# APRIL-ZJU/Gaussian-LIC

Measured on AMD Instinct MI355X. Metric: rendered views/sec (fwd+bwd) at 1080p, 2M Gaussians, higher is better.
Workload: dtype f32; 1 GPU; BASELINE config 3: 2000000 Gaussians (random scene, seed 0), 1920x1080, SH degree 3, render fwd + 0.8*L1+0.2*(1-fused-SSIM) + bwd + sparse Adam per view (fused entry points: activations and loss inside the kernels); learning rates x0.01 (stationary synthetic scene); map rows kept in Morton order by the library (bit-identical results; `insertion_order` beside it with --extras); mode=train, parallelism=single, math=strict, map_order=morton, binning=atomic (auto)

## Files before the change

### gaussian-lic_amd/_lib.py

```python
import ctypes
import os

import torch

_HERE = os.path.dirname(os.path.abspath(__file__))
LIB_PATH = os.environ.get("GSLIC_HIP_LIB") or os.path.join(_HERE, "libgslic_hip.so")

ALLOC_FN = ctypes.CFUNCTYPE(ctypes.c_void_p, ctypes.c_void_p, ctypes.c_size_t)


class RasterParams(ctypes.Structure):
    _fields_ = [("P", ctypes.c_int32), ("D", ctypes.c_int32), ("M", ctypes.c_int32), ("width", ctypes.c_int32),
                ("height", ctypes.c_int32), ("tan_fovx", ctypes.c_float), ("tan_fovy", ctypes.c_float),
                ("limx_neg", ctypes.c_float), ("limx_pos", ctypes.c_float), ("limy_neg", ctypes.c_float),
                ("limy_pos", ctypes.c_float), ("scale_modifier", ctypes.c_float), ("prefiltered", ctypes.c_int32),
                ("debug", ctypes.c_int32), ("no_color", ctypes.c_int32), ("raw_params", ctypes.c_int32), ("tie_rank", ctypes.c_void_p)]


class AdamGroup(ctypes.Structure):
    _fields_ = [("param", ctypes.c_void_p), ("grad", ctypes.c_void_p), ("exp_avg", ctypes.c_void_p),
                ("exp_avg_sq", ctypes.c_void_p), ("lr", ctypes.c_float), ("M", ctypes.c_uint32)]


class RowArray(ctypes.Structure):
    _fields_ = [("src", ctypes.c_void_p), ("dst", ctypes.c_void_p), ("row_dwords", ctypes.c_uint32)]


class AdamFused(ctypes.Structure):
    _fields_ = [("param", ctypes.c_void_p * 6), ("exp_avg", ctypes.c_void_p * 6), ("exp_avg_sq", ctypes.c_void_p * 6),
                ("lr", ctypes.c_float * 6), ("b1", ctypes.c_float), ("b2", ctypes.c_float), ("eps", ctypes.c_float), ("visible_out", ctypes.c_void_p)]


class GradStats(ctypes.Structure):
    _fields_ = [("grad_sum", ctypes.c_void_p), ("n_seen", ctypes.c_void_p), ("max_radius", ctypes.c_void_p)]


class ExposureAdam(ctypes.Structure):
    _fields_ = [("param", ctypes.c_void_p), ("m", ctypes.c_void_p), ("v", ctypes.c_void_p), ("step_count", ctypes.c_void_p), ("view", ctypes.c_void_p),
                ("lr", ctypes.c_float), ("beta1", ctypes.c_float), ("beta2", ctypes.c_float), ("eps", ctypes.c_float), ("skip", ctypes.c_void_p)]


EXPORTS = [
    "gslic_rasterize_forward", "gslic_rasterize_backward", "gslic_rasterize_backward_adam", "gslic_rasterize_backward_camera", "gslic_adam_update", "gslic_adam_update_groups",
    "gslic_fusedssim_forward", "gslic_fusedssim_backward", "gslic_knn_mean_dist2", "gslic_abi_version",
    "gslic_last_error", "gslic_geom_bytes", "gslic_img_bytes", "gslic_binning_bytes", "gslic_sample_bytes",
    "gslic_profile_enable", "gslic_profile_reset", "gslic_profile_collect", "gslic_profile_num_kernels",
    "gslic_profile_kernel_name", "gslic_profile_get", "gslic_debug_export", "gslic_extend_select", "gslic_extend_emit", "gslic_loss_partials_count", "gslic_l1_ssim_loss_forward", "gslic_l1_ssim_loss_forward_backward",
    "gslic_l1_ssim_loss_backward", "gslic_set_math_mode", "gslic_set_binning_mode", "gslic_rasterize_forward_capacity", "gslic_rasterize_backward_rgb",
    "gslic_rasterize_backward_rgb_rows", "gslic_sh_grad_from_rgb", "gslic_sh_grad_from_rgb_adam", "gslic_rasterize_backward_rgb_payload",
    "gslic_sh_grad_from_rgb_adam_all", "gslic_get_binning_path", "gslic_scratch_round_up",
    "gslic_rasterize_forward_depth", "gslic_rasterize_backward_depth",
    "gslic_rasterize_forward_depth_capacity", "gslic_rasterize_backward_depth_adam", "gslic_depth_l1_loss_partials_count",
    "gslic_depth_l1_loss_forward_backward", "gslic_img_bytes_depth", "gslic_binning_bytes_depth", "gslic_sample_bytes_depth",
    "gslic_rasterize_backward_depth_camera", "gslic_prune_select", "gslic_gather_rows", "gslic_contribution_accumulate",
    "gslic_contribution_accumulate_error", "gslic_contribution_accumulate_free_space", "gslic_densify_select", "gslic_densify_emit",
    "gslic_l1_ssim_loss_weighted_partials_count", "gslic_l1_ssim_loss_weighted_forward_backward",
    "gslic_morton_order", "gslic_permute_rows", "gslic_permute_rows_staging_bytes",
    "gslic_rasterize_backward_adam_stats", "gslic_rasterize_backward_depth_adam_stats", "gslic_gradient_stats_accumulate",
    "gslic_lidar_zbuffer_add", "gslic_lidar_zbuffer_resolve", "gslic_lidar_zbuffer_resolve_weighted",
    "gslic_depth_loss_weighted_partials_count", "gslic_depth_loss_weighted_forward_backward",
    "gslic_geometry_images",
    "gslic_exposure_partials_count", "gslic_exposure_apply", "gslic_exposure_backward",
    "gslic_keyframe_decode", "gslic_keyframe_encode",
]

_lib = None


class GslicError(RuntimeError):
    pass


def lib():
    global _lib
    if _lib is not None:
        return _lib
    if not os.path.exists(LIB_PATH):
        raise GslicError(f"{LIB_PATH} is missing: run `python gaussian-lic_amd/build.py` (hipcc, gfx950). "
                         "There is no CPU fallback.")
    L = ctypes.CDLL(LIB_PATH, mode=ctypes.RTLD_GLOBAL)
    vp, i32, f32, u32 = ctypes.c_void_p, ctypes.c_int32, ctypes.c_float, ctypes.c_uint32
    L.gslic_last_error.restype = ctypes.c_char_p
    L.gslic_profile_kernel_name.restype = ctypes.c_char_p
    L.gslic_profile_kernel_name.argtypes = [i32]
    L.gslic_profile_get.argtypes = [i32, ctypes.POINTER(ctypes.c_double), ctypes.POINTER(ctypes.c_int64)]
    for n in ("gslic_geom_bytes", "gslic_img_bytes", "gslic_binning_bytes", "gslic_sample_bytes", "gslic_img_bytes_depth", "gslic_binning_bytes_depth",
              "gslic_sample_bytes_depth"):
        getattr(L, n).restype = ctypes.c_size_t
    L.gslic_geom_bytes.argtypes = [i32]
    L.gslic_img_bytes.argtypes = [i32, i32]
    L.gslic_binning_bytes.argtypes = [i32, i32]
    L.gslic_sample_bytes.argtypes = [i32]
    L.gslic_img_bytes_depth.argtypes = [i32, i32]
    L.gslic_binning_bytes_depth.argtypes = [i32]
    L.gslic_sample_bytes_depth.argtypes = [i32]
    L.gslic_depth_l1_loss_partials_count.restype = ctypes.c_int64
    L.gslic_depth_l1_loss_partials_count.argtypes = [i32, i32]
    L.gslic_depth_l1_loss_forward_backward.argtypes = [i32, i32, f32, vp, vp, vp, vp, vp, vp]
    L.gslic_depth_loss_weighted_partials_count.restype = ctypes.c_int64
    L.gslic_depth_loss_weighted_partials_count.argtypes = [i32, i32]
    L.gslic_depth_loss_weighted_forward_backward.argtypes = [i32, i32, f32, f32] + [vp] * 6 + [vp]
    L.gslic_exposure_partials_count.restype = ctypes.c_int64
    L.gslic_exposure_partials_count.argtypes = [i32, i32]
    L.gslic_exposure_apply.argtypes = [i32, i32, vp, vp, vp, vp]
    L.gslic_exposure_backward.argtypes = [i32, i32] + [vp] * 6 + [ctypes.POINTER(ExposureAdam), vp]
    L.gslic_keyframe_decode.argtypes = [i32, i32, i32, vp, vp, vp, i32, vp, vp, vp]
    L.gslic_keyframe_encode.argtypes = [i32, i32, vp, vp, vp, vp, i32, i32, vp]
    prm, counts, adam = ctypes.POINTER(RasterParams), [ctypes.POINTER(i32), ctypes.POINTER(i32)], ctypes.POINTER(AdamFused)
    inputs = [vp] * 12
    fwd_head = [prm] + [ALLOC_FN, vp] * 4 + inputs
    cap_head = [prm] + [vp, ctypes.c_size_t] * 4 + inputs
    bwd_head = [prm, i32, i32] + inputs + [vp] * 4
    ten, six, five = [vp] * 10 + [f32], [vp] * 6 + [f32], [vp] * 5 + [f32]
    L.gslic_rasterize_forward.argtypes = fwd_head + [vp] * 3 + counts + [vp]
    L.gslic_rasterize_forward_depth.argtypes = fwd_head + [vp] * 4 + counts + [vp]
    L.gslic_rasterize_forward_capacity.argtypes = cap_head + [vp] * 3 + counts + [vp, vp]
    L.gslic_rasterize_forward_depth_capacity.argtypes = cap_head + [vp] * 4 + counts + [vp, vp]
    L.gslic_rasterize_backward.argtypes = bwd_head + [vp] + ten + [vp]
    L.gslic_rasterize_backward_depth.argtypes = bwd_head + [vp, vp] + ten + [vp]
    L.gslic_rasterize_backward_adam.argtypes = bwd_head + [vp] + six + [adam, vp]
    L.gslic_rasterize_backward_depth_adam.argtypes = bwd_head + [vp, vp] + six + [adam, vp]
    gstats = ctypes.POINTER(GradStats)
    L.gslic_rasterize_backward_adam_stats.argtypes = bwd_head + [vp] + six + [adam, gstats, vp]
    L.gslic_rasterize_backward_depth_adam_stats.argtypes = bwd_head + [vp, vp] + six + [adam, gstats, vp]
    L.gslic_gradient_stats_accumulate.argtypes = [i32, vp, vp, gstats, i32, i32, vp]
    L.gslic_rasterize_backward_camera.argtypes = bwd_head + [vp] + ten + [vp] * 3 + [vp]
    L.gslic_rasterize_backward_depth_camera.argtypes = bwd_head + [vp, vp] + ten + [vp] * 3 + [vp]
    L.gslic_rasterize_backward_rgb.argtypes = bwd_head + [vp] + five + [vp]
    L.gslic_rasterize_backward_rgb_rows.argtypes = bwd_head + [vp] + five + [i32, i32, i32, vp]
    L.gslic_rasterize_backward_rgb_payload.argtypes = bwd_head + [vp] + five + [vp, vp, vp]
    L.gslic_sh_grad_from_rgb_adam_all.argtypes = [i32, i32, i32, i32, vp, vp, vp, i32, vp, ctypes.c_int64, vp, ctypes.POINTER(AdamFused), vp, vp, vp, vp,
                                                  ctypes.c_int64, vp]
    L.gslic_sh_grad_from_rgb.argtypes = [i32, i32, i32, i32, vp, vp, vp, i32, vp, vp, ctypes.c_int64, vp]
    L.gslic_sh_grad_from_rgb_adam.argtypes = [i32, i32, i32, i32, vp, vp, vp, i32, vp, ctypes.POINTER(AdamFused), vp, vp, ctypes.c_int64, vp]
    L.gslic_adam_update.argtypes = [vp, vp, vp, vp, vp, f32, f32, f32, f32, u32, u32, vp]
    L.gslic_adam_update_groups.argtypes = [ctypes.POINTER(AdamGroup), i32, vp, f32, f32, f32, u32, vp]
    L.gslic_fusedssim_forward.argtypes = [i32, i32, i32, i32, f32, f32] + [vp] * 6 + [vp]
    L.gslic_fusedssim_backward.argtypes = [i32, i32, i32, i32, f32, f32] + [vp] * 7 + [vp]
    L.gslic_knn_mean_dist2.argtypes = [i32, vp, vp, ALLOC_FN, vp, vp]
    L.gslic_extend_select.argtypes = [i32, vp, vp, vp, vp, f32, f32, f32, f32, i32, i32, vp, ALLOC_FN, vp,
                                      ctypes.POINTER(vp), ctypes.POINTER(vp), ctypes.POINTER(i32), vp]
    L.gslic_extend_emit.argtypes = [i32, vp, vp, vp, vp, vp, f32, f32, i32, vp, vp, vp, vp, vp, vp, vp]
    L.gslic_prune_select.argtypes = [i32, vp, vp, vp, vp, vp, f32, f32, i32, vp, vp, vp, i32, ALLOC_FN, vp, vp, vp,
                                     ctypes.POINTER(i32), ctypes.POINTER(i32), vp]
    L.gslic_gather_rows.argtypes = [ctypes.POINTER(RowArray), i32, vp, i32, vp]
    L.gslic_lidar_zbuffer_add.argtypes = [i32, vp, vp, vp, f32, f32, f32, f32, i32, i32, vp, i32, i32, vp]
    L.gslic_lidar_zbuffer_resolve.argtypes = [i32, i32, vp, i32, f32, f32, vp, vp, vp, vp, vp]
    L.gslic_lidar_zbuffer_resolve_weighted.argtypes = [i32, i32, vp, i32, f32, f32, f32, f32, f32, vp, vp, vp, vp, vp, vp, vp]
    L.gslic_morton_order.argtypes = [i32, vp, vp, ALLOC_FN, vp, vp, vp, vp]
    L.gslic_permute_rows.argtypes = [ctypes.POINTER(RowArray), i32, vp, i32, vp, ctypes.c_size_t, vp]
    L.gslic_permute_rows_staging_bytes.restype = ctypes.c_size_t
    L.gslic_permute_rows_staging_bytes.argtypes = [ctypes.POINTER(RowArray), i32, i32]
    L.gslic_contribution_accumulate.argtypes = [prm, i32, i32, vp, vp, vp, f32, vp, vp, vp, vp]
    L.gslic_contribution_accumulate_error.argtypes = [prm, i32, i32, vp, vp, vp, f32, vp, vp, vp, vp, vp, vp]
    L.gslic_contribution_accumulate_free_space.argtypes = [prm, i32, i32, vp, vp, vp, f32, vp, vp, vp, vp, vp, vp, vp]
    L.gslic_geometry_images.argtypes = [prm, i32, i32, vp, vp, vp, f32] + [vp] * 7 + [vp]
    L.gslic_densify_select.argtypes = [i32, vp, vp, vp, vp, vp, vp, vp, vp, f32, ALLOC_FN, vp, vp, ctypes.POINTER(i32), ctypes.POINTER(i32), vp]
    six_ptrs = ctypes.POINTER(vp)
    L.gslic_densify_emit.argtypes = [i32, i32, vp, i32, six_ptrs, six_ptrs, six_ptrs, vp, f32, u32, vp]
    L.gslic_debug_export.argtypes = [ctypes.POINTER(RasterParams), i32, i32] + [vp] * 4 + [vp] * 10 + [vp]
    L.gslic_loss_partials_count.restype = ctypes.c_int64
    L.gslic_loss_partials_count.argtypes = [i32, i32, i32, i32]
    L.gslic_l1_ssim_loss_forward.argtypes = [i32, i32, i32, i32, f32, f32] + [vp] * 7 + [vp]
    L.gslic_l1_ssim_loss_backward.argtypes = [i32, i32, i32, i32, f32] + [vp] * 6 + [vp]
    L.gslic_l1_ssim_loss_forward_backward.argtypes = [i32, i32, i32, i32, f32, f32, f32] + [vp] * 8 + [vp]
    L.gslic_l1_ssim_loss_weighted_partials_count.restype = ctypes.c_int64
    L.gslic_l1_ssim_loss_weighted_partials_count.argtypes = [i32, i32, i32]
    L.gslic_l1_ssim_loss_weighted_forward_backward.argtypes = [i32, i32, i32, f32, f32, f32] + [vp] * 9 + [vp]
    L.gslic_set_math_mode.argtypes = [i32]
    L.gslic_set_binning_mode.argtypes = [i32]
    L.gslic_get_binning_path.argtypes = [ctypes.POINTER(u32), ctypes.POINTER(u32)]
    L.gslic_scratch_round_up.restype = ctypes.c_size_t
    L.gslic_scratch_round_up.argtypes = [ctypes.c_size_t]
    if L.gslic_abi_version() != 8:
        raise GslicError("libgslic_hip.so ABI version mismatch")
    _lib = L
    return L


def set_math_mode(strict):
    return bool(lib().gslic_set_math_mode(int(bool(strict))))


def set_binning_mode(mode):
    names = ("auto", "radix", "atomic")
    return names[lib().gslic_set_binning_mode(names.index(mode))]


def binning_path():
    a, n = ctypes.c_uint32(0), ctypes.c_uint32(0)
    path = lib().gslic_get_binning_path(ctypes.byref(a), ctypes.byref(n))
    return ("none", "radix", "atomic")[path], a.value, n.value


def check(rc):
    if rc != 0:
        raise GslicError(f"libgslic_hip error {rc}: {lib().gslic_last_error().decode()}")


def ptr(t):
    if t is None or t.numel() == 0:
        return None
    return ctypes.c_void_p(t.data_ptr())


def current_stream_ptr():
    return ctypes.c_void_p(torch.cuda.current_stream().cuda_stream)


class _AllocBox:
    __slots__ = ("device", "tensor", "__weakref__")

    def __init__(self, device):
# ... 57 lines not shown
```

### gaussian-lic_amd/csrc/api.hip

```cpp
#include "gslic_common.h"
#include "kernels.h"
#include <atomic>
#include <chrono>
#include <cmath>
#include <mutex>

#include <stdarg.h>
#include <stdio.h>
#include <stdlib.h>
#include <string.h>
#include <vector>

namespace gslic {

static thread_local char g_err[512] = "";
int set_error(int code, const char* fmt, ...)
{
    va_list ap;
    va_start(ap, fmt);
    vsnprintf(g_err, sizeof(g_err), fmt, ap);
    va_end(ap);
    return code;
}

// ... 506 lines not shown
        if (use_bin) {
            TileBinArgs tb;
            tb.T = T; tb.n_cap = R; tb.n_dev = R_dev; tb.tile = ka.tile_keys; tb.gid = ka.gauss; tb.depth = ka.depth; tb.tie_rank = prm->tie_rank;
            tb.ranges = img.ranges; tb.binned = bin.binned(); tb.dead = bin.dead; tb.status = geom.flags;
            tb.bucket_offsets = no_color ? nullptr : img.bucket_offsets; tb.max_contrib = img.max_contrib;
            ts.long_tiles = reinterpret_cast<uint32_t*>(bin.sort_scratch);
            GS_TRY(launch_tile_bin(tb, s));
            DEBUG_SYNC(prm, s);
            ts.binned = bin.binned(); ts.depth = nullptr; ts.gauss_in = nullptr; ts.slot_in = nullptr;
            ts.key_a = bin.tile_keys[0]; ts.key_b = bin.tile_keys[1]; ts.idx_a = bin.gauss[pp]; ts.idx_b = bin.slots[pp];
        } else {
            SortBuffers sb;
            for (int i = 0; i < 2; i++) { sb.keys[i] = bin.tile_keys[i]; sb.v0[i] = bin.slots[i]; sb.v1[i] = bin.gauss[i]; sb.v2[i] = bin.lsort[i]; }
            sb.v0_identity = true;
            GS_TRY(radix_sort_u32(sb, bin.plan, bin.sort_scratch, (onesweep_mask() & 2) != 0, K_SORT_HIST, K_SORT_SCATTER, s, R_dev, geom.flags + GS_FLAG_FAULT));
            DEBUG_SYNC(prm, s);
            GS_TRY(launch_finalize_ranges(R, R_dev, bin.tile_keys[pp], img.ranges, bin.dead, s));
            DEBUG_SYNC(prm, s);
            ts.binned = nullptr; ts.depth = bin.lsort[pp]; ts.gauss_in = bin.gauss[pp]; ts.slot_in = bin.slots[pp];
            ts.key_a = bin.lsort[pp ^ 1]; ts.key_b = bin.tile_keys[pp ^ 1]; ts.idx_a = bin.lsort[2]; ts.idx_b = bin.lsort[3];
        }
        GS_TRY(launch_tile_depth_sort(ts, s));
        DEBUG_SYNC(prm, s);
    }

    SampleState smp;
    memset(&smp, 0, sizeof(smp));
    uint32_t B = 0;
    if (!no_color) {
        if (!use_bin) GS_TRY(launch_bucket_scan(T, img.ranges, img.bucket_offsets, img.max_contrib, s));
        if (cap) {
            B = capacity_for(cap->sample_bytes, [&](uint32_t b) { size_t n; SampleState::carve(nullptr, (size_t)b, &n, depth); return n; });
        } else {
            uint32_t bin_sample[2] = {0, 0};
            GS_TRY(fetch_counts(img.bucket_offsets + (T - 1), nullptr, hostbuf, s, geom.flags + GS_FLAG_FAULT,
                                use_bin ? geom.flags + GS_FLAG_BIN_ATOMICS : nullptr, bin_sample));
            if (hostbuf[1] & 2u) return set_error(GSLIC_ERR_HIP, "a sort look-back / chained-scan wait timed out (device preempted?): the forward was abandoned");
            B = hostbuf[0];
            binning_feedback(prm->tie_rank != nullptr, use_bin, bin_sample[0], bin_sample[1]);
        }
        size_t smp_bytes;
        SampleState::carve(nullptr, (size_t)B, &smp_bytes, depth);
        char* smp_base = cap ? cap->sample : c.sample_alloc(c.sample_ctx, smp_bytes);
        if (!smp_base) return set_error(GSLIC_ERR_ALLOC, "sample allocator returned NULL for %zu bytes", smp_bytes);
        smp = SampleState::carve(align256(smp_base), (size_t)B, nullptr, depth);
    }

    RenderFwdArgs ra;
    ra.W = prm->width; ra.H = prm->height; ra.gx = gx; ra.gy = gy; ra.no_color = prm->no_color;
    ra.ranges = img.ranges; ra.point_list = bin.point_list(); ra.rec = geom.rec; ra.bucket_offsets = img.bucket_offsets;
    ra.bucket_to_tile = smp.bucket_to_tile; ra.ckpt = smp.ckpt; ra.hit = smp.hit; ra.pix_final = img.pix_final; ra.max_contrib = img.max_contrib;
    ra.out_color = c.out_color; ra.out_final_T = c.out_final_T; ra.capB = B; ra.status = geom.flags; ra.tail4_from = T;
    ra.out_depth = depth ? c.out_depth : nullptr; ra.ckpt_depth = smp.ckpt_depth; ra.pix_depth = img.pix_depth;
    GS_TRY(launch_render_fwd(ra, s));
    note_depth(geom.flags, depth);
    DEBUG_SYNC(prm, s);
    if (cap) {
        hipLaunchKernelGGL(forward_status_kernel, dim3(1), dim3(1), 0, s, (const uint32_t*)(geom.point_offsets + (P - 1)),
                           no_color ? (const uint32_t*)nullptr : (const uint32_t*)(img.bucket_offsets + (T - 1)), geom.flags, geom.flags + GS_FLAG_FAULT,
                           cap->status_out);
        GS_HIP(hipGetLastError());
    }

    *c.num_rendered = (int32_t)R;
    *c.num_buckets = (int32_t)B;
    return GSLIC_OK;
}

extern "C" {
int gslic_set_binning_mode(int32_t mode)
{
    if (mode < 0 || mode > 2) return g_binning_mode.load(std::memory_order_relaxed);
    const int old = g_binning_mode.exchange(mode, std::memory_order_relaxed);
    g_binning_epoch.fetch_add(1u, std::memory_order_release);
    return old;
}
int gslic_get_binning_path(uint32_t* sampled_atomics, uint32_t* sampled_instances)
{
    if (sampled_atomics) *sampled_atomics = t_last_sample[0];
    if (sampled_instances) *sampled_instances = t_last_sample[1];
    return t_last_path;
}
size_t gslic_scratch_round_up(size_t n)
{
    if (n <= (size_t(1) << 20)) return n;
    size_t g = size_t(32) << 20;
    if (n > (size_t(64) << 20)) {
        size_t p = 1;
        while ((p << 1) <= n && (p << 1) != 0) p <<= 1;
        const size_t half = p >> 1, cap = size_t(256) << 20;
        g = half > cap ? cap : (half > g ? half : g);
    }
    return (n + g - 1) / g * g;
}
#define GS_FORWARD_SHARED(c)                                                                                                               \
    c.prm = prm; c.means3D = means3D; c.dc = dc; c.shs = shs; c.colors_precomp = colors_precomp; c.opacities = opacities; c.scales = scales;       \
    c.rotations = rotations; c.cov3D_precomp = cov3D_precomp; c.viewmatrix = viewmatrix; c.projmatrix = projmatrix; c.cam_pos = cam_pos;           \
    c.out_color = out_color; c.out_final_T = out_final_T; c.radii = radii; c.stream = stream
#define GS_FORWARD_ALLOCATORS(c)                                                                                                           \
    c.geom_alloc = geom_alloc; c.geom_ctx = geom_ctx; c.binning_alloc = binning_alloc; c.binning_ctx = binning_ctx; c.img_alloc = img_alloc;       \
    c.img_ctx = img_ctx; c.sample_alloc = sample_alloc; c.sample_ctx = sample_ctx; c.num_rendered = num_rendered; c.num_buckets = num_buckets
#define GS_FORWARD_CAPACITY(c, cap)                                                                                                        \
    const ForwardCapacity cap{geom_buffer, binning_buffer, img_buffer, sample_buffer, geom_bytes, binning_bytes, img_bytes, sample_bytes, status}; \
    c.cap = &cap; c.num_rendered = capacity_R; c.num_buckets = capacity_B

int gslic_rasterize_forward(const gslic_raster_params* prm, gslic_alloc_fn geom_alloc, void* geom_ctx, gslic_alloc_fn binning_alloc,
// ... 1092 lines not shown
    if (o_depth) o_depth[i] = r2.y;
    if (o_co) { o_co[4 * i] = r0.z; o_co[4 * i + 1] = r0.w; o_co[4 * i + 2] = r1.x; o_co[4 * i + 3] = r1.y; }
    if (o_rgb) { o_rgb[3 * i] = r1.z; o_rgb[3 * i + 1] = r1.w; o_rgb[3 * i + 2] = r2.x; }
}
__global__ __launch_bounds__(256) void export_keys_kernel(uint32_t R, const uint2* __restrict__ ranges, const uint32_t* __restrict__ point_list,
                                                          const float4* __restrict__ rec, uint64_t* __restrict__ o)
{
    const uint2 r = ranges[blockIdx.x];
    for (uint32_t k = r.x + threadIdx.x; k < r.y && k < R; k += 256u)
        o[k] = ((uint64_t)blockIdx.x << 32) | __float_as_uint(rec[GS_REC_F4 * (size_t)point_list[k] + 2].y);
}
__global__ __launch_bounds__(256) void export_ncontrib_kernel(int W, int H, int gx, const float4* __restrict__ pix_final, uint32_t* o)
{
    const int x = blockIdx.x * 16 + (threadIdx.x & 15), y = blockIdx.y * 16 + (threadIdx.x >> 4);
    if (x >= W || y >= H) return;
    const int tile = blockIdx.y * gx + blockIdx.x;
    o[(size_t)y * W + x] = __float_as_uint(pix_final[(size_t)tile * GS_TILE_PIX + tile_pix_index((int)(threadIdx.x & 15), (int)(threadIdx.x >> 4))].w);
}
}

extern "C" int gslic_debug_export(const gslic_raster_params* prm, int32_t R, int32_t B, const char* geom_buffer,
                                  const char* binning_buffer, const char* img_buffer, const char* sample_buffer,
                                  uint32_t* tiles_touched, float* means2D, float* depths, float* conic_opacity, float* rgb,
                                  uint64_t* sorted_keys, uint32_t* point_list, uint32_t* ranges, uint32_t* n_contrib,
                                  uint32_t* max_contrib, void* stream)
{
    (void)B; (void)sample_buffer;
    GS_TRY(check_params(prm));
    hipStream_t s = (hipStream_t)stream;
    const int P = prm->P;
    int gx, gy;
    const int T = tile_grid(prm->width, prm->height, gx, gy);
    if (P == 0) return GSLIC_OK;
    GeomState geom = GeomState::carve(align256(const_cast<char*>(geom_buffer)), (size_t)P, nullptr);
    ImageState img = ImageState::carve(align256(const_cast<char*>(img_buffer)), (size_t)T, nullptr);
    BinningState bin = BinningState::carve(align256(const_cast<char*>(binning_buffer)), (size_t)R, sort_end_bit(T), prm->no_color != 0, nullptr);
    if (tiles_touched || means2D || depths || conic_opacity || rgb)
        GS_LAUNCH(K_DEBUG_EXPORT, export_geom_kernel, dim3(div_up(P, 256)), dim3(256), 0, s, P, (const float4*)geom.rec,
                  (const uint32_t*)geom.tiles_touched, tiles_touched, means2D, depths, conic_opacity, rgb);
    if (R > 0 && sorted_keys)
        GS_LAUNCH(K_DEBUG_EXPORT, export_keys_kernel, dim3((unsigned)T), dim3(256), 0, s, (uint32_t)R,
                  (const uint2*)img.ranges, (const uint32_t*)bin.point_list(), (const float4*)geom.rec, sorted_keys);
    if (R > 0 && point_list)
        GS_HIP(hipMemcpyAsync(point_list, bin.point_list(), (size_t)R * sizeof(uint32_t), hipMemcpyDeviceToDevice, s));
    if (ranges) GS_HIP(hipMemcpyAsync(ranges, img.ranges, (size_t)T * sizeof(uint2), hipMemcpyDeviceToDevice, s));
    if (!prm->no_color) {
        if (max_contrib) GS_HIP(hipMemcpyAsync(max_contrib, img.max_contrib, (size_t)T * sizeof(uint32_t), hipMemcpyDeviceToDevice, s));
        if (n_contrib)
            GS_LAUNCH(K_DEBUG_EXPORT, export_ncontrib_kernel, dim3(gx, gy), dim3(256), 0, s, prm->width, prm->height, gx,
                      (const float4*)img.pix_final, n_contrib);
    }
    return GSLIC_OK;
}
```

### gaussian-lic_amd/csrc/kernels.h

```cpp
#pragma once
#include "gslic_common.h"

namespace gslic {

struct PreprocessArgs {
    int P, D, M, W, H, gx, gy;
    float focal_x, focal_y;
    float limx_neg, limx_pos, limy_neg, limy_pos, scale_modifier;
    int prefiltered, no_color, raw;
    const float *means, *scales, *rots, *opac, *dc, *shs, *view, *proj, *campos;
    int32_t* radii;
    float4* rec;
    uint32_t* tiles_touched;
    uint32_t* depth_keys;
    uint2* ranges;
    uint32_t* flags;
};
int launch_preprocess(const PreprocessArgs& a, hipStream_t s);

struct KeybuildArgs {
    int P, gx, gy;
    const float4* rec;
    const uint32_t* order;
    const uint32_t* offsets;
    uint32_t* tile_keys;
    uint32_t* gauss;
    uint32_t* depth;
    uint32_t* gauss_start;
    uint32_t cap;
    uint32_t* status;
};
int launch_keybuild(const KeybuildArgs& a, hipStream_t s);
int launch_finalize_ranges(uint32_t R, const uint32_t* R_dev, const uint32_t* sorted_tiles, uint2* ranges, uint8_t* dead, hipStream_t s);
int launch_bucket_scan(int T, const uint2* ranges, uint32_t* bucket_offsets, uint32_t* max_contrib , hipStream_t s);

struct RenderFwdArgs {
    int W, H, gx, gy, no_color;
    const uint2* ranges;
    const uint32_t* point_list;
    const float4* rec;
    const uint32_t* bucket_offsets;
    uint32_t* bucket_to_tile;
    float4* ckpt;
    uint64_t* hit;
    float4* pix_final;
    uint32_t* max_contrib;
    float* out_color;
    float* out_final_T;
    uint32_t capB;
    uint32_t* status;
    int tail4_from;
    float* out_depth;
    float* ckpt_depth;
    float* pix_depth;
};
int launch_render_fwd(const RenderFwdArgs& a, hipStream_t s);

struct RenderBwdArgs {
    int W, H, gx, B;
    const uint2* ranges;
    const uint32_t* point_list;
    const uint32_t* inst_slot;
    const float4* rec;
    const uint32_t* bucket_offsets;
    const uint32_t* bucket_to_tile;
    const float4* ckpt;
    const uint64_t* hit;
    const float4* pix_final;
    const uint32_t* max_contrib;
    const float* dL_dpix;
    float* partials;
    uint8_t* dead;
    const uint32_t* status;
    int T;
    int xcd_lg;
    int skip_if_bits;
    const float* dL_ddepth;
    const float* ckpt_depth;
    const float* pix_depth;
    float* partials_z;
};
int launch_render_bwd(const RenderBwdArgs& a, hipStream_t s);
int launch_render_bwd_scan(const RenderBwdArgs& b, unsigned grid, hipStream_t s);

struct AdamFusedArgs {
    float *p[6], *m[6], *v[6];
    float lr[6];
    float b1, b2, eps;
    int on;
};

struct PreprocessBwdArgs {
    int P, D, M, W, H, raw;
    int row_begin, row_end;
    float focal_x, focal_y;
    float limx_neg, limx_pos, limy_neg, limy_pos, scale_modifier, lambda_erank;
    const float *means, *scales, *rots, *dc, *shs, *view, *proj, *campos;
    const int32_t* radii;
    const float4* rec;
    const uint32_t* tiles_touched;
    const uint32_t* gauss_start;
    const float* partials;
    const uint8_t* dead;
    float *dL_dmean2D, *dL_dconic, *dL_dopacity, *dL_dcolor, *dL_dmean3D, *dL_dcov3D, *dL_ddc, *dL_dsh, *dL_dscale, *dL_drot;
    float* dL_drgb;
    AdamFusedArgs adam;
    const uint32_t* status;
// ... 114 lines not shown
```

### gaussian-lic_amd/csrc/render.hip

```cpp
#include "gslic_common.h"
#include "kernels.h"
#include <stdlib.h>
#include <mutex>

namespace gslic {

__device__ __forceinline__ float strip_max_p2(float hA, float hC, float nB, float gx, float gy, float x0, float x1, float y0, float y1)
{
    const bool in_x = gx >= x0 && gx <= x1, in_y = gy >= y0 && gy <= y1;
    if (in_x && in_y) return 0.0f;
    float best = -3.0e38f;
    if (!in_y) {
        const float ye = gy < y0 ? y0 : y1;
        const float dy = gy - ye;
        float dx = -(nB * dy) / (2.0f * hA);
        dx = fminf(fmaxf(dx, gx - x1), gx - x0);
        best = fmaxf(best, (hA * dx) * dx + (hC * dy) * dy + (nB * dx) * dy);
    }
    if (!in_x) {
        const float xe = gx < x0 ? x0 : x1;
        const float dx = gx - xe;
        float dy = -(nB * dx) / (2.0f * hC);
        dy = fminf(fmaxf(dy, gy - y1), gy - y0);
        best = fmaxf(best, (hA * dx) * dx + (hC * dy) * dy + (nB * dx) * dy);
// ... 96 lines not shown
            asm("v_bfi_b32 %0, %1, %2, %3" : "=v"(sel_) : "v"(klo), "v"(GH.x), "v"(GH.y));                            \
            asm("v_bfe_i32 %0, %1, %2, 1" : "=v"(m_) : "v"(sel_), "v"(kbit));                                         \
            ah = __uint_as_float(__float_as_uint(araw) & m_);                                                        \
        } else {  \
            const bool hit = (kcmp < TAG) & !(p2 > L.lop) & !(araw < c255);                                          \
            ah = hit ? araw : 0.0f;                                                                                  \
        }                                                                                                            \
        const float alpha = __builtin_amdgcn_fmed3f(ah, ninf, c099);  \
        const float om = 1.0f - alpha;                                                                               \
        const float rinv = __builtin_amdgcn_rcpf(om);    \
        const float Ta = T_ * alpha;                                                                                 \
        float cg = L.col_rg.x * gr.x;                                                                                \
        cg = __builtin_fmaf(L.col_rg.y, gr.y, cg);                                                                   \
        cg = __builtin_fmaf(L.colb, gr.z, cg);                                                    \
        if (DEPTH) { cg = __builtin_fmaf(L.z, GD, cg);                        \
                     acc_z = __builtin_fmaf(Ta, GD, acc_z); }                                                        \
        acc_rg = GS_PK_FMA(GS_SPLAT(Ta), ((v2f){gr.x, gr.y}), acc_rg); acc_b = __builtin_fmaf(Ta, gr.z, acc_b);      \
        A_ = __builtin_fmaf(Ta, cg, A_);                                                                             \
        const float dLda = __builtin_fmaf(rinv, A_, T_ * cg);                                                        \
        T_ *= om;                                                                                                    \
        const float w = ah * dLda;          \
        const v2f wd = GS_SPLAT(w) * d;                                                                              \
        acc_S += wd;                                                                                                 \
        acc_cxy = GS_PK_FMA(GS_SPLAT(wd.x), d, acc_cxy);                                \
        acc_cw = __builtin_fmaf(wd.y, d.y, acc_cw);                                                                  \
        acc_op += w;                                                          \
    } while (0)

template <bool BITS, bool DEPTH>
__global__ __launch_bounds__(64) void render_bwd_kernel(RenderBwdArgs a)
{
    constexpr int NENT = GS_TILE_PIX + 1;
    constexpr uint32_t BW_OFF_BT = NENT * 8u, BW_OFF_TA = 2u * NENT * 8u, BW_OFF_HM = 3u * NENT * 8u, BW_OFF_GD = (BITS ? 4u : 3u) * NENT * 8u;
    __shared__ float2 smem[((BITS ? 4 : 3) + (DEPTH ? 1 : 0)) * NENT];
    float2* const s_rg = smem;
    float2* const s_bt = smem + NENT;
    float2* const s_ta = smem + 2 * NENT;
    uint2* const s_hm = reinterpret_cast<uint2*>(smem + 3 * NENT);
    float2* const s_gd = smem + (BITS ? 4 : 3) * NENT;
    const int lane = threadIdx.x;
    uint32_t bucket = blockIdx.x;
    if (a.xcd_lg >= 0) {
        const uint32_t x = bucket & 7u, j = bucket >> 3;
        bucket = ((((j >> a.xcd_lg) << 3) + x) << a.xcd_lg) + (j & ((1u << a.xcd_lg) - 1u));
    }
    if (a.status[2] != 0u || bucket >= a.bucket_offsets[a.T - 1]) return;
    const bool use_bits = BITS && a.status[GS_FLAG_HITBITS] != 0u;
    if (a.skip_if_bits && use_bits) return;
    const uint32_t tile = a.bucket_to_tile[bucket];
    const uint2 range = a.ranges[tile];
    const uint32_t n = range.y - range.x;
    const uint32_t bbm = (tile == 0) ? 0u : a.bucket_offsets[tile - 1];
    const uint32_t bstart = (bucket - bbm) * GS_BUCKET;
    const uint32_t kit = bstart + (uint32_t)lane;
    const bool valid = kit < n;
    const uint32_t slot = valid ? a.inst_slot[range.x + kit] : 0u;

    if (bstart >= a.max_contrib[tile]) {
        if (valid) a.dead[slot] = 1;
        return;
    }

    const int tx0 = (int)(tile % (uint32_t)a.gx) * GS_TILE, ty0 = (int)(tile / (uint32_t)a.gx) * GS_TILE;
    const size_t plane = (size_t)a.H * a.W;
    float4 ck[4], pf[4];
    float fg[4][3], ckd[4], pfd[4], fgd[4];
    bool inside[4];
    uint2 hm[4];
#pragma unroll
    for (int c = 0; c < 4; c++) {
        const int pidx = c * 64 + lane;
        ck[c] = a.ckpt[(size_t)bucket * GS_TILE_PIX + pidx];
        hm[c] = make_uint2(0u, 0u);
        if constexpr (BITS) {
            if (use_bits) { const uint64_t m = a.hit[(size_t)bucket * GS_TILE_PIX + pidx]; hm[c] = make_uint2((uint32_t)m, (uint32_t)(m >> 32)); }
        }
        pf[c] = a.pix_final[(size_t)tile * GS_TILE_PIX + pidx];
        const int px = tx0 + tile_pix_x(pidx), py = ty0 + tile_pix_y(pidx);
        inside[c] = px < a.W && py < a.H;
        fg[c][0] = fg[c][1] = fg[c][2] = 0.f;
        ckd[c] = pfd[c] = fgd[c] = 0.f;
        if constexpr (DEPTH) { ckd[c] = a.ckpt_depth[(size_t)bucket * GS_TILE_PIX + pidx]; pfd[c] = a.pix_depth[(size_t)tile * GS_TILE_PIX + pidx]; }
        if (inside[c]) {
            const size_t pid = (size_t)py * a.W + px;
            fg[c][0] = a.dL_dpix[pid]; fg[c][1] = a.dL_dpix[plane + pid]; fg[c][2] = a.dL_dpix[2 * plane + pid];
            if constexpr (DEPTH) fgd[c] = a.dL_ddepth[pid];
        }
    }
    const float LOG2E = 1.4426950408889634f;
    BwdLane L;
    L.d0 = L.hAC = L.col_rg = (v2f){0.f, 0.f};
    L.nB = L.colb = L.z = 0.f;
    L.lop = -__builtin_inff();
    float rop = 0.f;
    if (valid) {
        const uint32_t g = a.point_list[range.x + kit];
        const float4* rp = a.rec + GS_REC_F4 * (size_t)g;
        const float4 r0 = rp[0], r1 = rp[1], r2 = rp[2];
        L.d0.x = r0.x - (float)tx0; L.d0.y = r0.y - (float)ty0;
        L.hAC.x = -0.5f * LOG2E * r0.z; L.nB = -LOG2E * r0.w; L.hAC.y = -0.5f * LOG2E * r1.x;
        L.lop = __builtin_amdgcn_logf(r1.y);
        rop = r1.y > 0.f ? 1.0f / r1.y : 0.f;
        L.col_rg.x = r1.z; L.col_rg.y = r1.w; L.colb = r2.x;
        if constexpr (DEPTH) L.z = r2.y;
    }

    uint32_t rel[4], key[4], pos[4];
    uint64_t cm[4][4];
    uint32_t ninj = 0;
#pragma unroll
    for (int c = 0; c < 4; c++) {
        const uint32_t ncp = inside[c] ? __float_as_uint(pf[c].w) : 0u;
        rel[c] = ncp > bstart ? (ncp - bstart < 64u ? ncp - bstart : 64u) : 0u;
        key[c] = rel[c] ? (rel[c] - 1u) >> 4 : 4u;
// ... 172 lines not shown
```

### gaussian-lic_amd/csrc/render_bwd_scan.hip

```cpp
#include "gslic_common.h"
#include "kernels.h"
#include <stdlib.h>

#ifndef GS_SCAN_SKIP
#define GS_SCAN_SKIP 0
#endif

namespace gslic {

typedef float v2f_s __attribute__((ext_vector_type(2)));

template <int CTRL, int ROW_MASK = 0xf>
__device__ __forceinline__ float dpp_f(float old, float src)
{
    return __int_as_float(__builtin_amdgcn_update_dpp(__float_as_int(old), __float_as_int(src), CTRL, ROW_MASK, 0xf, false));
}
template <int CTRL, int ROW_MASK = 0xf>
__device__ __forceinline__ uint32_t dpp_u(uint32_t old, uint32_t src)
{
    return (uint32_t)__builtin_amdgcn_update_dpp((int)old, (int)src, CTRL, ROW_MASK, 0xf, false);
}
#ifdef GS_SCAN_SAFE
__device__ __forceinline__ float row_scan_mul(float x)
{
// ... 149 lines not shown
            const v2f_s wd = (v2f_s){w, w} * d;
            acc_S[g] += wd;
            acc_cxy[g] = __builtin_elementwise_fma((v2f_s){wd.x, wd.x}, d, acc_cxy[g]);
            acc_cw[g] = __builtin_fmaf(wd.y, dy, acc_cw[g]);
            acc_op[g] += w;
            if (g + 1 < NG) { Tin = row_last(Tincl); Ain = row_last(Ap); }
        }
    }
#pragma unroll
    for (int g = 0; g < NG; g++) {
        float v[9] = {acc_S[g].x, acc_S[g].y, acc_cxy[g].x, acc_cxy[g].y, acc_cw[g], acc_op[g], acc_rg[g].x, acc_rg[g].y, acc_b[g]};
#pragma unroll
        for (int k = 0; k < 9; k++) {
            v[k] += __shfl_xor(v[k], 16, 64);
            v[k] += __shfl_xor(v[k], 32, 64);
        }
        if (row == 0 && 16 * g + slot_i < ne) {
#pragma unroll
            for (int k = 0; k < 9; k++) S.acc[9 * ent[g] + k] += v[k];
        }
        if constexpr (DEPTH) {
            float vz = acc_z[g];
            vz += __shfl_xor(vz, 16, 64);
            vz += __shfl_xor(vz, 32, 64);
            if (row == 0 && 16 * g + slot_i < ne) accz[ent[g]] += vz;
        }
    }
}

#ifndef GS_SCAN_WAVES
#define GS_SCAN_WAVES 4
#endif
#ifndef GS_SCAN_WAVES_DEPTH
#define GS_SCAN_WAVES_DEPTH GS_SCAN_WAVES
#endif
template <bool DEPTH>
__global__ __launch_bounds__(64, DEPTH ? GS_SCAN_WAVES_DEPTH : GS_SCAN_WAVES) void render_bwd_scan_kernel(RenderBwdArgs a)
{
    __shared__ ScanLds S;
    __shared__ float s_accz[DEPTH ? 64 : 1];
    const int lane = threadIdx.x;
    uint32_t bucket = blockIdx.x;
    if (a.xcd_lg >= 0) {
        const uint32_t x = bucket & 7u, j = bucket >> 3;
        bucket = ((((j >> a.xcd_lg) << 3) + x) << a.xcd_lg) + (j & ((1u << a.xcd_lg) - 1u));
    }
    if (a.status[2] != 0u || bucket >= a.bucket_offsets[a.T - 1]) return;
    if (a.status[GS_FLAG_HITBITS] == 0u) return;
    const uint32_t tile = a.bucket_to_tile[bucket];
    const uint2 range = a.ranges[tile];
    const uint32_t n = range.y - range.x;
    const uint32_t bbm = (tile == 0) ? 0u : a.bucket_offsets[tile - 1];
    const uint32_t bstart = (bucket - bbm) * GS_BUCKET;
    const uint32_t kit = bstart + (uint32_t)lane;
    const bool valid = kit < n;
    const uint32_t slot = valid ? a.inst_slot[range.x + kit] : 0u;
    if (bstart >= a.max_contrib[tile]) {
        if (valid && !((GS_SCAN_SKIP & 8) && a.T > -1)) a.dead[slot] = 1;
        return;
    }
    const int tx0 = (int)(tile % (uint32_t)a.gx) * GS_TILE, ty0 = (int)(tile / (uint32_t)a.gx) * GS_TILE;
    const size_t plane = (size_t)a.H * a.W;

    const float LOG2E = 1.4426950408889634f;
    {
    ScanEntry L = {0.f, 0.f, 0.f, 0.f, 0.f, -__builtin_inff(), 0.f, 0.f, 0.f, 0.f};
    float rop = 0.f;
    if (valid && !((GS_SCAN_SKIP & 32) && a.T > -1)) {
        const uint32_t g = a.point_list[range.x + kit];
        const float4* rp = a.rec + GS_REC_F4 * (size_t)g;
        const float4 r0 = rp[0], r1 = rp[1], r2 = rp[2];
        L.d0x = r0.x - (float)tx0; L.d0y = r0.y - (float)ty0;
        L.hA = -0.5f * LOG2E * r0.z; L.nB = -LOG2E * r0.w; L.hC = -0.5f * LOG2E * r1.x;
        L.lop = __builtin_amdgcn_logf(r1.y);
        rop = r1.y > 0.f ? 1.0f / r1.y : 0.f;
        L.cr = r1.z; L.cg = r1.w; L.cb = r2.x;
        if constexpr (DEPTH) L.z = r2.y;
    }
    S.ent[SC_ENT_F4 * lane] = make_float4(L.d0x, L.d0y, L.hA, L.hC);
    S.ent[SC_ENT_F4 * lane + 1] = make_float4(L.nB, L.lop, L.cr, L.cg);
    S.ent[SC_ENT_F4 * lane + 2] = make_float4(L.cb, rop, __uint_as_float(slot), DEPTH ? L.z : 0.f);
#pragma unroll
    for (int k = 0; k < 9; k++) S.acc[9 * lane + k] = 0.f;
    if constexpr (DEPTH) s_accz[lane] = 0.f;
    }

    float c099 = 0.99f;
    asm volatile("" : "+v"(c099));

    struct PixIn { uint64_t hm; float4 pf, ck; float g0, g1, g2, ckd, pfd, gd; };
    auto load_pix = [&](int q) {
        PixIn r;
        const int pidx = q * 64 + lane;
        r.hm = a.hit[(size_t)bucket * GS_TILE_PIX + pidx];
        r.pf = a.pix_final[(size_t)tile * GS_TILE_PIX + pidx];
        r.ck = a.ckpt[(size_t)bucket * GS_TILE_PIX + pidx];
        const int px = tx0 + tile_pix_x(pidx), py = ty0 + tile_pix_y(pidx);
        r.g0 = r.g1 = r.g2 = 0.f;
        r.ckd = r.pfd = r.gd = 0.f;
        if constexpr (DEPTH) { r.ckd = a.ckpt_depth[(size_t)bucket * GS_TILE_PIX + pidx]; r.pfd = a.pix_depth[(size_t)tile * GS_TILE_PIX + pidx]; }
        if (px < a.W && py < a.H) {
            const size_t pid = (size_t)py * a.W + px;
            r.g0 = a.dL_dpix[pid]; r.g1 = a.dL_dpix[plane + pid]; r.g2 = a.dL_dpix[2 * plane + pid];
            if constexpr (DEPTH) r.gd = a.dL_ddepth[pid];
        }
        return r;
    };
#ifndef GS_SCAN_PREFETCH
#define GS_SCAN_PREFETCH 0
#endif
#if GS_SCAN_PREFETCH
    PixIn nxt = load_pix(0);
#endif
// ... 99 lines not shown
```

### gaussian-lic_amd/csrc/render_fwd_body.inc

```
{
    constexpr int QN = 4 / GS_BODY_SPLIT;
    const int lane = threadIdx.x;
    const int tx0 = (tile % a.gx) * GS_TILE, ty0 = (tile / a.gx) * GS_TILE;
    if (a.status[2] != 0u) return;
    if (STRICT && !a.no_color && blockIdx.x == 0 && lane == 0) a.status[GS_FLAG_HITBITS] = 1u;
    if (DEPTH && blockIdx.x == 0 && lane == 0) a.status[GS_FLAG_DEPTH] = 1u;
    const uint2 range = a.ranges[tile];
    const int n = (int)(range.y - range.x);
    const bool color = !a.no_color;

    uint32_t bbm = 0;
    bool fits = true;
    if (color) {
        bbm = (tile == 0) ? 0u : a.bucket_offsets[tile - 1];
        const int nb = (n + GS_BUCKET - 1) / GS_BUCKET;
        fits = bbm + (uint32_t)nb <= a.capB;
        if (!fits && lane == 0) atomicOr(a.status + 2, 2u);
        if (fits && q0 == 0)
            for (int b = lane; b < nb; b += 64) a.bucket_to_tile[bbm + b] = (uint32_t)tile;
    }

    constexpr int MY = QN == 4 ? 2 : 1;
    int pxi[QN], pyi[QN];
#pragma unroll
// ... 142 lines not shown
        };
        float4 a0 = s_rec[0], a1 = s_rec[1], a2 = s_rec[2], b0, b1, b2;
        for (int j = 0; j < (((GS_FWD_SKIP & 1) && a.gx > -1) ? 0 : m); j += 2) {
            if constexpr (STRICT) {
                if (j == 32) {
#pragma unroll
                    for (int q = 0; q < QN; q++) { hfirst[q] = hcur[q]; hcur[q] = 0u; }
                }
            }
            const int jb = (j + 1 < m) ? j + 1 : j;
            b0 = s_rec[3 * jb]; b1 = s_rec[3 * jb + 1]; b2 = s_rec[3 * jb + 2];
            blend_entry(a0, a1, a2, (uint32_t)(base + j + 1));
            if (j + 1 >= m) break;
            const int ja = (j + 2 < m) ? j + 2 : j;
            a0 = s_rec[3 * ja]; a1 = s_rec[3 * ja + 1]; a2 = s_rec[3 * ja + 2];
            blend_entry(b0, b1, b2, (uint32_t)(base + j + 2));
        }
        if constexpr (STRICT) {
            if (color && fits && !((GS_FWD_SKIP & 4) && a.gx > -1)) {
                uint64_t* hp = a.hit + ((size_t)(bbm + (uint32_t)(base / GS_BUCKET)) * GS_TILE_PIX) + lane;
#pragma unroll
                for (int q = 0; q < QN; q++)
                    hp[(q0 + q) * 64] = m > 32 ? (((uint64_t)hcur[q] << 32) | hfirst[q]) : (uint64_t)hcur[q];
            }
        }
    }

    uint32_t mymax = 0;
    const size_t plane = (size_t)a.H * a.W;
#pragma unroll
    for (int q = 0; q < QN; q++) {
        if (pxi[q] < a.W && pyi[q] < a.H) {
            const size_t pid = (size_t)pyi[q] * a.W + pxi[q];
            a.out_final_T[pid] = fabsf(T[q]);
            if (color) {
                a.out_color[pid] = Cr[q];
                a.out_color[plane + pid] = Cg[q];
                a.out_color[2 * plane + pid] = Cb[q];
            }
            if constexpr (DEPTH) a.out_depth[pid] = Dz[q];
        }
        if (color) {
            a.pix_final[(size_t)tile * GS_TILE_PIX + (q0 + q) * 64 + lane] = make_float4(Cr[q], Cg[q], Cb[q], __uint_as_float(last[q]));
            if constexpr (DEPTH) a.pix_depth[(size_t)tile * GS_TILE_PIX + (q0 + q) * 64 + lane] = Dz[q];
            mymax = last[q] > mymax ? last[q] : mymax;
        }
    }
    if (color) {
#pragma unroll
        for (int d = 32; d >= 1; d >>= 1) {
            const uint32_t o = (uint32_t)__shfl_xor((int)mymax, d, 64);
            mymax = o > mymax ? o : mymax;
        }
        if (lane == 0) {
            if constexpr (GS_BODY_SPLIT == 1) a.max_contrib[tile] = mymax;
            else atomicMax(a.max_contrib + tile, mymax);
        }
    }
}
```

### gaussian-lic_amd/rasterizer.py

```python
import ctypes
from dataclasses import dataclass

import torch

from . import _lib


@dataclass
class GaussianRasterizationSettings:
    image_height: int
    image_width: int
    tanfovx: float
    tanfovy: float
    limx_neg: float
    limx_pos: float
    limy_neg: float
    limy_pos: float
    bg: torch.Tensor
    scale_modifier: float
    viewmatrix: torch.Tensor
    projmatrix: torch.Tensor
    sh_degree: int
    campos: torch.Tensor
    prefiltered: bool = False
# ... 463 lines not shown
                                                        bp(n_pix), bp(sum_w), _lib.current_stream_ptr()))


GEOMETRY_IMAGES = ("transmittance", "opacity", "depth_sum", "depth_norm", "depth_median", "top_row", "top_weight")


def geometry_images(P, H, W, R, B, geom, binning, img, a_min, out):
    unknown = set(out) - set(GEOMETRY_IMAGES)
    if unknown:
        raise ValueError(f"geometry_images: unknown image(s) {sorted(unknown)}; the images are {GEOMETRY_IMAGES}")
    ptrs = []
    for name in GEOMETRY_IMAGES:
        t = out.get(name)
        dt = torch.int32 if name == "top_row" else torch.float32
        if t is not None and not (torch.is_tensor(t) and t.is_contiguous() and t.dtype == dt and t.numel() == int(H) * int(W) and t.numel() > 0):
            raise ValueError(f"geometry_images: {name} must be a contiguous {dt} tensor of {int(H)} x {int(W)} elements")
        ptrs.append(None if t is None else ctypes.c_void_p(t.data_ptr()))
    prm = _params(P, 0, 0, H, W, 1.0, 1.0, 0.0, 0.0, 0.0, 0.0, 1.0, False, False, False)
    bp = lambda t: ctypes.c_void_p(t.data_ptr()) if t is not None and t.numel() else None
    _lib.check(_lib.lib().gslic_geometry_images(ctypes.byref(prm), int(R), int(B), bp(geom), bp(binning), bp(img), float(a_min), *ptrs,
                                                _lib.current_stream_ptr()))


def debug_export(settings, P, M, R, B, geom, binning, img, sample, what=("tiles_touched", "point_list", "ranges")):
    L = _lib.lib()
    rs = settings
    dev = geom.device
    H, W = rs.image_height, rs.image_width
    T = ((W + 15) // 16) * ((H + 15) // 16)
    prm = _params(P, rs.sh_degree, M, H, W, rs.tanfovx, rs.tanfovy, rs.limx_neg, rs.limx_pos, rs.limy_neg, rs.limy_pos,
                  rs.scale_modifier, False, False, rs.no_color)
    out = {}
    mk = dict(
        tiles_touched=lambda: torch.zeros(P, dtype=torch.int32, device=dev),
        means2D=lambda: torch.zeros(P, 2, device=dev), depths=lambda: torch.zeros(P, device=dev),
        conic_opacity=lambda: torch.zeros(P, 4, device=dev), rgb=lambda: torch.zeros(P, 3, device=dev),
        sorted_keys=lambda: torch.zeros(max(R, 1), dtype=torch.int64, device=dev),
        point_list=lambda: torch.zeros(max(R, 1), dtype=torch.int32, device=dev),
        ranges=lambda: torch.zeros(T, 2, dtype=torch.int32, device=dev),
        n_contrib=lambda: torch.zeros(H, W, dtype=torch.int32, device=dev),
        max_contrib=lambda: torch.zeros(T, dtype=torch.int32, device=dev))
    order = ["tiles_touched", "means2D", "depths", "conic_opacity", "rgb", "sorted_keys", "point_list", "ranges", "n_contrib",
             "max_contrib"]
    args = []
    for k in order:
        if k in what:
            out[k] = mk[k]()
            args.append(ctypes.c_void_p(out[k].data_ptr()))
        else:
            args.append(None)
    bp = lambda t: ctypes.c_void_p(t.data_ptr()) if t.numel() else None
    _lib.check(L.gslic_debug_export(ctypes.byref(prm), int(R), int(B), bp(geom), bp(binning), bp(img), bp(sample), *args,
                                    _lib.current_stream_ptr()))
    torch.cuda.synchronize()
    for k in ("sorted_keys", "point_list"):
        if k in out:
            out[k] = out[k][:R]
    return out
```

### include/gslic_hip.h

```cpp
#ifndef GSLIC_HIP_H_INCLUDED
#define GSLIC_HIP_H_INCLUDED

#include <stddef.h>
#include <stdint.h>

#ifdef __cplusplus
extern "C" {
#endif

#define GSLIC_ABI_VERSION 8

typedef enum gslic_status {
    GSLIC_OK = 0,
    GSLIC_ERR_INVALID_ARG = -1,
    GSLIC_ERR_UNSUPPORTED = -2,
    GSLIC_ERR_ALLOC = -3,
    GSLIC_ERR_HIP = -4,
    GSLIC_ERR_PREFILTERED = -5
} gslic_status;

typedef char* (*gslic_alloc_fn)(void* ctx, size_t bytes);

typedef struct gslic_raster_params {
    int32_t P;
// ... 400 lines not shown
    const gslic_raster_params* prm, int32_t R, int32_t B,
    const char* geom_buffer, const char* binning_buffer, const char* img_buffer, float a_min,
    float* transmittance, float* opacity, float* depth_sum, float* depth_norm, float* depth_median,
    int32_t* top_row, float* top_weight , void* stream);

int gslic_densify_select(
    int32_t P, const float* xyz, const float* dc, const float* opacity_raw, const float* scaling_raw, const float* rotation_raw,
    const uint8_t* grow , const uint8_t* protect , const uint32_t* tie_rank , float scaling_raw_split,
    gslic_alloc_fn scratch_alloc, void* scratch_ctx,
    uint32_t* parent_index , int32_t* count, int32_t* count_split, void* stream);
int gslic_densify_emit(
    int32_t P, int32_t count, const uint32_t* parent_index, int32_t M,
    float* const param[6], float* const exp_avg[6], float* const exp_avg_sq[6],
    uint32_t* tie_rank , float scaling_raw_split, uint32_t seed, void* stream);

int gslic_abi_version(void);
const char* gslic_last_error(void);

int gslic_set_math_mode(int32_t strict);

int gslic_set_binning_mode(int32_t mode);

#define GSLIC_BINNING_PATH_NONE 0
#define GSLIC_BINNING_PATH_RADIX 1
#define GSLIC_BINNING_PATH_ATOMIC 2
int gslic_get_binning_path(uint32_t* sampled_atomics, uint32_t* sampled_instances);

size_t gslic_scratch_round_up(size_t bytes);

size_t gslic_geom_bytes(int32_t P);
size_t gslic_img_bytes(int32_t width, int32_t height);
size_t gslic_binning_bytes(int32_t R, int32_t no_color);
size_t gslic_sample_bytes(int32_t B);
size_t gslic_img_bytes_depth(int32_t width, int32_t height);
size_t gslic_binning_bytes_depth(int32_t R);
size_t gslic_sample_bytes_depth(int32_t B);

#define GSLIC_PROFILE_MAX_KERNELS 48
int gslic_profile_enable(int32_t on);
int gslic_profile_reset(void);
int gslic_profile_collect(void);
int gslic_profile_num_kernels(void);
const char* gslic_profile_kernel_name(int32_t id);
int gslic_profile_get(int32_t id, double* total_ms, int64_t* launches);

int gslic_debug_export(
    const gslic_raster_params* prm, int32_t R, int32_t B,
    const char* geom_buffer, const char* binning_buffer, const char* img_buffer, const char* sample_buffer,
    uint32_t* tiles_touched , float* means2D , float* depths ,
    float* conic_opacity , float* rgb ,
    uint64_t* sorted_keys , uint32_t* point_list , uint32_t* ranges ,
    uint32_t* n_contrib , uint32_t* max_contrib ,
    void* stream);

#ifdef __cplusplus
}
#endif
#endif
```

Baseline: 572.5 views/s.

## Mark dead tail instances in forward render instead of backward bucket kernels

Moves the marking of Gaussian instances beyond each tile's last contributor from the backward bucket kernels into the forward render. When split across bodies, the last finisher is found with a CAS counter packed into the upper bits of max_contrib. Backward buckets past max_contrib now return at once, without loading inst_slot or writing dead flags. This adds a CAS loop and a strided scatter in the forward pass. Packing a counter into max_contrib relies on the value fitting in 30 bits and on the final writer clearing the count. A debug export for inst_slot, dead and hit buffers is also added.

```diff
diff --git a/gaussian-lic_amd/_lib.py b/gaussian-lic_amd/_lib.py
--- a/gaussian-lic_amd/_lib.py
+++ b/gaussian-lic_amd/_lib.py
@@ -62,6 +62,7 @@
     "gslic_geometry_images",
     "gslic_exposure_partials_count", "gslic_exposure_apply", "gslic_exposure_backward",
     "gslic_keyframe_decode", "gslic_keyframe_encode",
+    "gslic_debug_export_flags",
 ]
 
 _lib = None
@@ -159,6 +160,7 @@
     six_ptrs = ctypes.POINTER(vp)
     L.gslic_densify_emit.argtypes = [i32, i32, vp, i32, six_ptrs, six_ptrs, six_ptrs, vp, f32, u32, vp]
     L.gslic_debug_export.argtypes = [ctypes.POINTER(RasterParams), i32, i32] + [vp] * 4 + [vp] * 10 + [vp]
+    L.gslic_debug_export_flags.argtypes = [ctypes.POINTER(RasterParams), i32, i32] + [vp] * 2 + [vp] * 3 + [vp]
     L.gslic_loss_partials_count.restype = ctypes.c_int64
     L.gslic_loss_partials_count.argtypes = [i32, i32, i32, i32]
     L.gslic_l1_ssim_loss_forward.argtypes = [i32, i32, i32, i32, f32, f32] + [vp] * 7 + [vp]
diff --git a/gaussian-lic_amd/csrc/api.hip b/gaussian-lic_amd/csrc/api.hip
--- a/gaussian-lic_amd/csrc/api.hip
+++ b/gaussian-lic_amd/csrc/api.hip
@@ -582,6 +582,7 @@
     ra.bucket_to_tile = smp.bucket_to_tile; ra.ckpt = smp.ckpt; ra.hit = smp.hit; ra.pix_final = img.pix_final; ra.max_contrib = img.max_contrib;
     ra.out_color = c.out_color; ra.out_final_T = c.out_final_T; ra.capB = B; ra.status = geom.flags; ra.tail4_from = T;
     ra.out_depth = depth ? c.out_depth : nullptr; ra.ckpt_depth = smp.ckpt_depth; ra.pix_depth = img.pix_depth;
+    ra.inst_slot = bin.inst_slot(); ra.dead = bin.dead;
     GS_TRY(launch_render_fwd(ra, s));
     note_depth(geom.flags, depth);
     DEBUG_SYNC(prm, s);
@@ -1780,3 +1781,19 @@
     }
     return GSLIC_OK;
 }
+
+extern "C" int gslic_debug_export_flags(const gslic_raster_params* prm, int32_t R, int32_t B, const char* binning_buffer, const char* sample_buffer,
+                                        uint32_t* inst_slot, uint8_t* dead, uint64_t* hit, void* stream)
+{
+    GS_TRY(check_params(prm));
+    hipStream_t s = (hipStream_t)stream;
+    int gx, gy;
+    const int T = tile_grid(prm->width, prm->height, gx, gy);
+    if (prm->P == 0 || prm->no_color) return GSLIC_OK;
+    BinningState bin = BinningState::carve(align256(const_cast<char*>(binning_buffer)), (size_t)R, sort_end_bit(T), false, nullptr);
+    SampleState smp = SampleState::carve(align256(const_cast<char*>(sample_buffer)), (size_t)B, nullptr, false);
+    if (R > 0 && inst_slot) GS_HIP(hipMemcpyAsync(inst_slot, bin.inst_slot(), (size_t)R * sizeof(uint32_t), hipMemcpyDeviceToDevice, s));
+    if (R > 0 && dead) GS_HIP(hipMemcpyAsync(dead, bin.dead, (size_t)R, hipMemcpyDeviceToDevice, s));
+    if (B > 0 && hit) GS_HIP(hipMemcpyAsync(hit, smp.hit, (size_t)B * GS_TILE_PIX * sizeof(uint64_t), hipMemcpyDeviceToDevice, s));
+    return GSLIC_OK;
+}
diff --git a/gaussian-lic_amd/csrc/kernels.h b/gaussian-lic_amd/csrc/kernels.h
--- a/gaussian-lic_amd/csrc/kernels.h
+++ b/gaussian-lic_amd/csrc/kernels.h
@@ -53,6 +53,8 @@
     float* out_depth;
     float* ckpt_depth;
     float* pix_depth;
+    const uint32_t* inst_slot;
+    uint8_t* dead;
 };
 int launch_render_fwd(const RenderFwdArgs& a, hipStream_t s);
 
diff --git a/gaussian-lic_amd/csrc/render.hip b/gaussian-lic_amd/csrc/render.hip
--- a/gaussian-lic_amd/csrc/render.hip
+++ b/gaussian-lic_amd/csrc/render.hip
@@ -172,14 +172,10 @@
     const uint32_t n = range.y - range.x;
     const uint32_t bbm = (tile == 0) ? 0u : a.bucket_offsets[tile - 1];
     const uint32_t bstart = (bucket - bbm) * GS_BUCKET;
+    if (bstart >= a.max_contrib[tile]) return;
     const uint32_t kit = bstart + (uint32_t)lane;
     const bool valid = kit < n;
     const uint32_t slot = valid ? a.inst_slot[range.x + kit] : 0u;
-
-    if (bstart >= a.max_contrib[tile]) {
-        if (valid) a.dead[slot] = 1;
-        return;
-    }
 
     const int tx0 = (int)(tile % (uint32_t)a.gx) * GS_TILE, ty0 = (int)(tile / (uint32_t)a.gx) * GS_TILE;
     const size_t plane = (size_t)a.H * a.W;
diff --git a/gaussian-lic_amd/csrc/render_bwd_scan.hip b/gaussian-lic_amd/csrc/render_bwd_scan.hip
--- a/gaussian-lic_amd/csrc/render_bwd_scan.hip
+++ b/gaussian-lic_amd/csrc/render_bwd_scan.hip
@@ -225,13 +225,10 @@
     const uint32_t n = range.y - range.x;
     const uint32_t bbm = (tile == 0) ? 0u : a.bucket_offsets[tile - 1];
     const uint32_t bstart = (bucket - bbm) * GS_BUCKET;
+    if (bstart >= a.max_contrib[tile]) return;
     const uint32_t kit = bstart + (uint32_t)lane;
     const bool valid = kit < n;
     const uint32_t slot = valid ? a.inst_slot[range.x + kit] : 0u;
-    if (bstart >= a.max_contrib[tile]) {
-        if (valid && !((GS_SCAN_SKIP & 8) && a.T > -1)) a.dead[slot] = 1;
-        return;
-    }
     const int tx0 = (int)(tile % (uint32_t)a.gx) * GS_TILE, ty0 = (int)(tile / (uint32_t)a.gx) * GS_TILE;
     const size_t plane = (size_t)a.H * a.W;
 
diff --git a/gaussian-lic_amd/csrc/render_fwd_body.inc b/gaussian-lic_amd/csrc/render_fwd_body.inc
--- a/gaussian-lic_amd/csrc/render_fwd_body.inc
+++ b/gaussian-lic_amd/csrc/render_fwd_body.inc
@@ -218,9 +218,34 @@
             const uint32_t o = (uint32_t)__shfl_xor((int)mymax, d, 64);
             mymax = o > mymax ? o : mymax;
         }
-        if (lane == 0) {
-            if constexpr (GS_BODY_SPLIT == 1) a.max_contrib[tile] = mymax;
-            else atomicMax(a.max_contrib + tile, mymax);
+        bool flagger = fits;
+        uint32_t mc = mymax;
+        if constexpr (GS_BODY_SPLIT == 1) {
+            if (lane == 0) a.max_contrib[tile] = mymax;
+        } else {
+            uint32_t done = 0u;
+            if (lane == 0) {
+                uint32_t old = 0u;
+                for (;;) {
+                    const uint32_t cnt = (old >> 30) + 1u, run = old & 0x3fffffffu, mx = run > mymax ? run : mymax;
+                    const uint32_t seen = atomicCAS(a.max_contrib + tile, old, cnt == (uint32_t)GS_BODY_SPLIT ? mx : ((cnt << 30) | mx));
+                    if (seen == old) { done = cnt == (uint32_t)GS_BODY_SPLIT ? 1u : 0u; mc = mx; break; }
+                    old = seen;
+                }
+            }
+            flagger = fits && __builtin_amdgcn_readfirstlane((int)done) != 0;
+            mc = (uint32_t)__builtin_amdgcn_readfirstlane((int)mc);
+        }
+        if (flagger && a.dead != nullptr) {
+            const uint32_t un = (uint32_t)n;
+            for (uint32_t p = ((mc + (uint32_t)(GS_BUCKET - 1)) & ~(uint32_t)(GS_BUCKET - 1)) + (uint32_t)lane; p < un; p += 4u * 64u) {
+                uint32_t sl[4];
+#pragma unroll
+                for (int k = 0; k < 4; k++) sl[k] = p + 64u * k < un ? a.inst_slot[range.x + p + 64u * k] : 0xffffffffu;
+#pragma unroll
+                for (int k = 0; k < 4; k++)
+                    if (sl[k] != 0xffffffffu) a.dead[sl[k]] = 1;
+            }
         }
     }
 }
diff --git a/gaussian-lic_amd/rasterizer.py b/gaussian-lic_amd/rasterizer.py
--- a/gaussian-lic_amd/rasterizer.py
+++ b/gaussian-lic_amd/rasterizer.py
@@ -539,6 +539,21 @@
     bp = lambda t: ctypes.c_void_p(t.data_ptr()) if t.numel() else None
     _lib.check(L.gslic_debug_export(ctypes.byref(prm), int(R), int(B), bp(geom), bp(binning), bp(img), bp(sample), *args,
                                     _lib.current_stream_ptr()))
+    mk2 = dict(inst_slot=lambda: torch.zeros(max(R, 1), dtype=torch.int32, device=dev),
+               dead=lambda: torch.zeros(max(R, 1), dtype=torch.uint8, device=dev),
+               hit=lambda: torch.zeros(max(B, 1), 256, dtype=torch.int64, device=dev))
+    if any(k in what for k in mk2):
+        args2 = []
+        for k in mk2:
+            if k in what:
+                out[k] = mk2[k]()
+                args2.append(ctypes.c_void_p(out[k].data_ptr()))
+            else:
+                args2.append(None)
+        _lib.check(L.gslic_debug_export_flags(ctypes.byref(prm), int(R), int(B), bp(binning), bp(sample), *args2, _lib.current_stream_ptr()))
+        for k, n in (("inst_slot", R), ("dead", R), ("hit", B)):
+            if k in out:
+                out[k] = out[k][:n]
     torch.cuda.synchronize()
     for k in ("sorted_keys", "point_list"):
         if k in out:
diff --git a/include/gslic_hip.h b/include/gslic_hip.h
--- a/include/gslic_hip.h
+++ b/include/gslic_hip.h
@@ -476,6 +476,9 @@
     uint64_t* sorted_keys , uint32_t* point_list , uint32_t* ranges ,
     uint32_t* n_contrib , uint32_t* max_contrib ,
     void* stream);
+int gslic_debug_export_flags(
+    const gslic_raster_params* prm, int32_t R, int32_t B, const char* binning_buffer, const char* sample_buffer,
+    uint32_t* inst_slot , uint8_t* dead , uint64_t* hit , void* stream);
 
 #ifdef __cplusplus
 }
```

New measurement: 571.5 views/s. No clear change (-0.2%).
